# endernewton/tf-faster-rcnn

Measured on AMD Instinct MI355X. Metric: images/sec (600×1000) ResNet-101 Faster R-CNN at 1/2/4/8 MI355X, higher is better.
Workload: dtype f32 (operands, accumulators, results; GEMMs with Cin, Cout % 128 == 0 form each f32 product from two-piece fp16 operands with an exact power-of-two scale per 128-k block on the fp16 matrix pipe -- 3 MFMAs / product, dropped terms <= 3 * 2^-22, measured error vs float64 below the f32-MFMA kernel's; o

## Files before the change

include/frcnn_hip.h:

```cpp
#ifndef FRCNN_HIP_H_
#define FRCNN_HIP_H_
#include <stddef.h>
#include <stdint.h>

#ifdef __cplusplus
extern "C" {
#endif

#define FRCNN_OK 0
#define FRCNN_E_ARG (-1)
#define FRCNN_E_WS (-2)
#define FRCNN_E_UNSUPPORTED (-3)
#define FRCNN_E_HIP(e) (-(1000 + (int)(e)))

#define FRCNN_NMS_RULE_CPU 0
#define FRCNN_NMS_RULE_GPU 1

#define FRCNN_ACT_NONE 0
#define FRCNN_ACT_RELU 1
#define FRCNN_ACT_RELU6 2

#define FRCNN_ABI_VERSION 6
int frcnn_abi_version(void);
const char* frcnn_build_info(void);
// ... 128 lines not shown

int frcnn_gemm_batched_nt(const float* x_d, const float* w_d, float* y_d, int G, int M, int N, int K, void* stream);
size_t frcnn_gemm_x3_pack_bytes(int G, int N, int K);
int frcnn_gemm_x3_pack(const float* w_d, int G, int N, int K, void* planes_d, void* stream);
int frcnn_gemm_x3(const float* x_d, const void* planes_d, const float* bias_d, const float* res_d, float* y_d, int G, int M, int N,
                  int K, int act, int cfg, int terms, void* stream);
size_t frcnn_h2_planes_bytes(long long rows, int K);
int frcnn_h2_pack_w(const float* w_d, int G, int N, int K, void* planes_d, float* w_inv_d, void* stream);
int frcnn_h2_split(const float* x_d, long long M, int K, void* planes_d, float* inv_d, void* stream);
int frcnn_gemm_h2(const void* x_planes_d, const float* x_inv_d, const void* w_planes_d, const float* w_inv_d, const float* bias_d,
                  const float* res_d, const void* res_planes_d, const float* res_inv_d, float* y_d, void* y_planes_d, float* y_inv_d,
                  int G, int M, int N, int K, int act, int cfg, void* stream);
size_t frcnn_gemm_h2_mean_workspace_bytes(int G, int M, int N);
int frcnn_gemm_h2_mean(const void* x_planes_d, const float* x_inv_d, const void* w_planes_d, const float* w_inv_d, const float* bias_d,
                       const float* res_d, const void* res_planes_d, const float* res_inv_d, int G, int M, int N, int K, int act, int rows,
                       float* mean_out_d, void* ws, size_t ws_bytes, int cfg, void* stream);
int frcnn_winograd_filter_transform(const float* w_hwio, int Cin, int Cout, const float* scale, int m, float* u_out);
int frcnn_winograd_filter_transform_device(const float* w_packed_d, int Cout, int Cin, int m, int transpose_flip, float* u_d,
                                           void* stream);
int frcnn_winograd_input_transform(const float* x_d, int N, int H, int W, int C, int m, float* v_d, void* stream);
int frcnn_winograd_output_transform(const float* m_d, int N, int H, int W, int C, int m, const float* bias_d, int act, float* y_d,
                                    void* stream);
int frcnn_winograd7_filter_transform(const float* w_hwio, int Cin, int Cout, const float* scale, float* u_out);
int frcnn_winograd7_filter_transform_device(const float* w_packed_d, int Cout, int Cin, int transpose_flip, float* u_d, void* stream);
int frcnn_winograd7_input_transform(const float* x_d, int R, int C, float* v_d, void* stream);
int frcnn_winograd7_output_transform(const float* m_d, int R, int C, const float* bias_d, int act, float* y_d, void* stream);
int frcnn_winograd_input_transform_h2(const float* x_d, int N, int H, int W, int C, int m, void* v_planes_d, float* v_inv_d, void* stream);
int frcnn_winograd_output_transform_h2(const float* m_d, int N, int H, int W, int C, int m, const float* bias_d, int act, float* y_d,
                                       void* y_planes_d, float* y_inv_d, void* stream);
int frcnn_winograd7_input_transform_h2(const float* x_d, int R, int C, void* v_planes_d, float* v_inv_d, void* stream);
int frcnn_winograd7_output_transform_h2(const float* m_d, int R, int C, const float* bias_d, int act, float* y_d, void* y_planes_d,
                                        float* y_inv_d, void* stream);
int frcnn_pack_filter_hwio(const float* w_hwio, int KH, int KW, int Cin, int Cout, const float* scale, float* out);
int frcnn_maxpool_nhwc(const float* x_d, int N, int H, int W, int C, int k, int stride, int pad_top,
                       int pad_left, float* y_d, int OH, int OW, void* stream);
int frcnn_dwconv3x3_nhwc(const float* x_d, int N, int H, int W, int C, const float* w_d, const float* bias_d,
                         float* y_d, int OH, int OW, int stride, int pad_top, int pad_left, int act, void* stream);
int frcnn_dwconv3x3_nhwc_h2(const float* x_d, int N, int H, int W, int C, const float* w_d, const float* bias_d, float* y_d,
                            void* y_planes_d, float* y_inv_d, int OH, int OW, int stride, int pad_top, int pad_left, int act, void* stream);
int frcnn_spatial_mean(const float* x_d, int N, int HW, int C, float* y_d, void* stream);
int frcnn_softmax_rows(const float* x_d, int R, int C, int ld, float* y_d, void* stream);
int frcnn_rpn_softmax(const float* score_d, int HW, int A, int ld, float* prob_d, void* stream);
int frcnn_copy_cols(const float* src_d, int R, int ld_src, int col0, int cols, float* dst_d, int ld_dst, void* stream);

size_t frcnn_anchor_target_workspace_bytes(int H, int W, int A, int max_gt);
int frcnn_anchor_target_layer(const float* gt_boxes_d, int G, float im_h, float im_w, int H, int W, int A,
                              int feat_stride, const double* base_d, int rpn_batchsize, double fg_fraction,
                              double pos_overlap, double neg_overlap, long long seed, const double* opts, float* labels_d,
                              float* bbox_targets_d, float* inside_w_d, float* outside_w_d, void* ws,
                              size_t ws_bytes, void* stream);
int frcnn_anchor_target_layer_inject(const float* gt_boxes_d, int G, float im_h, float im_w, int H, int W, int A, int feat_stride,
                                     const double* base_d, int rpn_batchsize, double fg_fraction, double pos_overlap,
                                     double neg_overlap, const int* disable_d, int n_disable, const double* opts, float* labels_d,
                                     float* bbox_targets_d, float* inside_w_d, float* outside_w_d, void* ws, size_t ws_bytes,
                                     void* stream);
int frcnn_proposal_target_layer(const float* rpn_rois_d, const float* rpn_scores_d, int N, const float* gt_boxes_d,
                                int G, int num_classes, int batch_size, double fg_fraction, double fg_thresh,
                                double bg_thresh_hi, double bg_thresh_lo, const double* means4, const double* stds4,
                                long long seed, const double* opts, float* rois_d, float* roi_scores_d, float* labels_d,
                                float* bbox_targets_d, float* inside_w_d, float* outside_w_d, int* counts_d,
                                void* stream);
int frcnn_proposal_target_layer_dn(const float* rpn_rois_d, const float* rpn_scores_d, int max_rois, const int* num_rois_d,
                                   const float* gt_boxes_d, int G, int num_classes, int batch_size, double fg_fraction,
                                   double fg_thresh, double bg_thresh_hi, double bg_thresh_lo, const double* means4,
                                   const double* stds4, long long seed, const double* opts, float* rois_d, float* roi_scores_d,
                                   float* labels_d, float* bbox_targets_d, float* inside_w_d, float* outside_w_d, int* counts_d,
// ... 90 lines not shown
```

tf-faster-rcnn_amd/frcnn_hip/__init__.py:

```python
import ctypes
import os
from ctypes import c_double, c_float, c_int, c_longlong, c_size_t, c_ulonglong, c_void_p

_PKG = os.path.dirname(os.path.abspath(__file__))
LIB_PATH = os.path.join(_PKG, "libfrcnn_hip.so")
_lib = None

ABI_VERSION = 6
ACT_NONE, ACT_RELU, ACT_RELU6 = 0, 1, 2
NMS_RULE_CPU, NMS_RULE_GPU = 0, 1

_P = c_void_p
SIGNATURES = {
    "frcnn_abi_version": (c_int, []),
    "frcnn_build_info": (ctypes.c_char_p, []),
    "_nms": (None, [_P, _P, _P, c_int, c_int, c_float, c_int]),
    "frcnn_nms_workspace_bytes": (c_size_t, [c_int]),
    "frcnn_nms": (c_int, [_P, c_int, c_double, c_int, _P, _P, _P, c_size_t, _P]),
    "frcnn_nms_sorted": (c_int, [_P, c_int, c_int, c_double, c_int, _P, _P, _P, c_size_t, _P]),
    "frcnn_nms_rule": (c_int, [_P, c_int, c_double, c_int, c_int, _P, _P, _P, c_size_t, _P]),
    "frcnn_nms_sorted_rule": (c_int, [_P, c_int, c_int, c_double, c_int, c_int, _P, _P, _P, c_size_t, _P]),
    "frcnn_generate_anchors": (c_int, [c_int, _P, c_int, _P, c_int, _P]),
    "frcnn_generate_anchors_pre": (c_int, [c_int, c_int, c_int, _P, c_int, _P, _P]),
    "frcnn_proposal_workspace_bytes": (c_size_t, [c_int, c_int, c_int, c_int]),
# ... 41 lines not shown
    "frcnn_snappy_uncompress": (c_longlong, [_P, c_size_t, _P, c_size_t]),
    "frcnn_prep_image_shape": (c_int, [c_int, c_int, c_int, c_int, _P, _P, _P]),
    "frcnn_prep_image": (c_int, [_P, c_int, c_int, c_int, _P, c_double, _P, c_int, c_int, c_int, _P]),
    "frcnn_prep_image_batched": (c_int, [_P, c_int, c_int, c_int, c_int, _P, c_double, _P, c_int, c_int, c_int, _P]),
    "frcnn_prep_train_image": (c_int, [_P, c_int, c_int, c_int, c_int, _P, c_double, _P, c_int, c_int, c_int, _P, _P, c_int, _P, _P]),
    "frcnn_jpeg_info": (c_int, [_P, c_size_t, _P]),
    "frcnn_jpeg_coef_bytes": (c_size_t, [c_int, c_int, c_int, c_int, c_int]),
    "frcnn_jpeg_entropy_decode": (c_int, [_P, c_size_t, _P, c_size_t]),
    "frcnn_jpeg_pixels_host": (c_int, [_P, c_int, c_int, c_int, c_int, c_int, _P]),
    "frcnn_jpeg_workspace_bytes": (c_size_t, [c_int, c_int, c_int, c_int, c_int]),
    "frcnn_jpeg_pixels": (c_int, [_P, c_int, c_int, c_int, c_int, c_int, _P, _P, c_size_t, _P]),
    "frcnn_jpeg_quant_tables": (c_int, [c_int, _P]),
    "frcnn_jpeg_coefs": (c_int, [_P, c_int, c_int, c_int, c_int, c_int, _P, _P, c_size_t, _P]),
    "frcnn_jpeg_coefs_host": (c_int, [_P, c_int, c_int, c_int, c_int, c_int, _P]),
    "frcnn_jpeg_stream_bound": (c_size_t, [c_int, c_int, c_int, c_int]),
    "frcnn_jpeg_entropy_encode": (c_longlong, [_P, c_int, c_int, c_int, c_int, _P, c_size_t]),
    "frcnn_draw_detections": (c_int, [_P, c_int, c_int, _P, _P, c_int, c_float, c_int, c_int, _P, c_int, _P, c_int, c_int, _P, _P]),
    "frcnn_draw_detections_host": (c_int, [_P, c_int, c_int, _P, c_int, c_int, c_float, c_int, c_int, _P, c_int, _P, c_int, c_int, _P]),
    "frcnn_gemm_batched_nt": (c_int,[_P, _P, _P, c_int, c_int, c_int, c_int, _P]),
    "frcnn_winograd_filter_transform": (c_int, [_P, c_int, c_int, _P, c_int, _P]),
    "frcnn_winograd_filter_transform_device": (c_int, [_P, c_int, c_int, c_int, c_int, _P, _P]),
    "frcnn_winograd_input_transform": (c_int, [_P, c_int, c_int, c_int, c_int, c_int, _P, _P]),
    "frcnn_winograd_output_transform": (c_int, [_P, c_int, c_int, c_int, c_int, c_int, _P, c_int, _P, _P]),
    "frcnn_winograd7_filter_transform": (c_int, [_P, c_int, c_int, _P, _P]),
    "frcnn_winograd7_filter_transform_device": (c_int, [_P, c_int, c_int, c_int, _P, _P]),
    "frcnn_winograd7_input_transform": (c_int, [_P, c_int, c_int, _P, _P]),
    "frcnn_winograd7_output_transform": (c_int, [_P, c_int, c_int, _P, c_int, _P, _P]),
    "frcnn_winograd_input_transform_h2": (c_int, [_P, c_int, c_int, c_int, c_int, c_int, _P, _P, _P]),
    "frcnn_winograd_output_transform_h2": (c_int, [_P, c_int, c_int, c_int, c_int, c_int, _P, c_int, _P, _P, _P, _P]),
    "frcnn_winograd7_input_transform_h2": (c_int, [_P, c_int, c_int, _P, _P, _P]),
    "frcnn_winograd7_output_transform_h2": (c_int, [_P, c_int, c_int, _P, c_int, _P, _P, _P, _P]),
    "frcnn_set_tuning": (c_int, [c_int, c_int]),
    "frcnn_pack_filter_hwio": (c_int, [_P, c_int, c_int, c_int, c_int, _P, _P]),
    "frcnn_maxpool_nhwc": (c_int, [_P, c_int, c_int, c_int, c_int, c_int, c_int, c_int, c_int, _P, c_int, c_int, _P]),
    "frcnn_dwconv3x3_nhwc": (c_int, [_P, c_int, c_int, c_int, c_int, _P, _P, _P, c_int, c_int, c_int, c_int, c_int, c_int, _P]),
    "frcnn_dwconv3x3_nhwc_h2": (c_int, [_P, c_int, c_int, c_int, c_int, _P, _P, _P, _P, _P, c_int, c_int, c_int, c_int, c_int, c_int, _P]),
    "frcnn_spatial_mean": (c_int, [_P, c_int, c_int, c_int, _P, _P]),
    "frcnn_softmax_rows": (c_int, [_P, c_int, c_int, c_int, _P, _P]),
    "frcnn_rpn_softmax": (c_int, [_P, c_int, c_int, c_int, _P, _P]),
    "frcnn_copy_cols": (c_int, [_P, c_int, c_int, c_int, c_int, _P, c_int, _P]),
    "frcnn_anchor_target_workspace_bytes": (c_size_t, [c_int, c_int, c_int, c_int]),
    "frcnn_anchor_target_layer": (c_int, [_P, c_int, c_float, c_float, c_int, c_int, c_int, c_int, _P, c_int, c_double, c_double,
                                          c_double, c_longlong, _P, _P, _P, _P, _P, _P, c_size_t, _P]),
    "frcnn_anchor_target_layer_inject": (c_int, [_P, c_int, c_float, c_float, c_int, c_int, c_int, c_int, _P, c_int, c_double, c_double,
                                                 c_double, _P, c_int, _P, _P, _P, _P, _P, _P, c_size_t, _P]),
    "frcnn_proposal_target_layer_inject": (c_int, [_P, _P, c_int, _P, c_int, c_int, c_int, _P, c_int, _P, _P, _P, _P, _P, _P, _P, _P, _P, _P]),
    "frcnn_proposal_target_layer": (c_int, [_P, _P, c_int, _P, c_int, c_int, c_int, c_double, c_double, c_double, c_double, _P, _P,
                                            c_longlong, _P, _P, _P, _P, _P, _P, _P, _P, _P]),
    "frcnn_proposal_target_layer_dn": (c_int, [_P, _P, c_int, _P, _P, c_int, c_int, c_int, c_double, c_double, c_double, c_double, _P, _P,
                                               c_longlong, _P, _P, _P, _P, _P, _P, _P, _P, _P]),
    "frcnn_loss_workspace_bytes": (c_size_t, [c_longlong]),
    "frcnn_softmax_ce_loss": (c_int, [_P, _P, c_int, c_int, c_int, c_int, c_int, _P, _P, _P, c_size_t, _P]),
    "frcnn_smooth_l1_loss": (c_int, [_P, _P, _P, _P, c_longlong, c_float, c_float, _P, _P, _P, c_size_t, _P]),
    "frcnn_transpose_pad": (c_int, [_P, c_int, c_int, _P, c_int, _P]),
    "frcnn_im2col_t": (c_int, [_P, c_int, c_int, c_int, c_int, c_int, c_int, c_int, c_int, c_int, c_int, c_int, _P, c_int, _P]),
    "frcnn_flip_transpose_filter": (c_int, [_P, c_int, c_int, c_int, c_int, _P, _P]),
    "frcnn_conv2d_dgrad_strided": (c_int, [_P, c_int, c_int, c_int, c_int, _P, c_int, c_int, c_int, c_int, c_int, c_int, _P, c_int,
                                           c_int, c_int, _P]),
    "frcnn_conv2d_wgrad_supported": (c_int, [c_int, c_int]),
    "frcnn_conv2d_wgrad_workspace_bytes": (c_size_t, [c_int, c_int, c_int, c_int, c_int, c_int, c_int]),
    "frcnn_conv2d_wgrad": (c_int, [_P, _P, c_int, c_int, c_int, c_int, c_int, c_int, c_int, c_int, c_int, c_int, c_int, c_int, _P, _P,
                                   c_size_t, _P]),
    "frcnn_conv2d_wgrad_set_plan": (None, [c_int, c_int]),
    "frcnn_conv2d_wgrad_h2_workspace_bytes": (c_size_t, [c_int, c_int, c_int, c_int, c_int, c_int, c_int]),
    "frcnn_conv2d_wgrad_h2": (c_int, [_P, _P, c_int, c_int, c_int, c_int, c_int, c_int, c_int, c_int, c_int, c_int, c_int, c_int, _P, _P,
                                      c_size_t, _P]),
# ... 78 lines not shown
```

tf-faster-rcnn_amd/frcnn_hip/build.py:

```python
import glob
import os
import subprocess
import sys
from concurrent.futures import ThreadPoolExecutor

PKG = os.path.dirname(os.path.abspath(__file__))
ROOT = os.path.dirname(os.path.dirname(PKG))
CSRC = os.path.join(os.path.dirname(PKG), "csrc")
OBJ = os.path.join(CSRC, "build")
LIB = os.path.join(PKG, "libfrcnn_hip.so")
SOURCES = ["detect_kernels.hip", "conv_igemm.hip", "dense_misc.hip", "train_kernels.hip", "backward_kernels.hip", "winograd.hip", "winograd7.hip", "preproc.hip", "gemm_x3.hip", "gemm_h2.hip", "wgrad_tn.hip", "wgrad_h2.hip", "coco_eval.hip", "jpeg_decode.hip", "summary_stats.hip", "jpeg_encode.hip", "draw.hip"]
FLAGS = ["-O3", "-std=c++17", "--offload-arch=gfx950", "-fPIC", "-ffp-contract=off",
         "-I" + os.path.join(ROOT, "include"), "-I" + CSRC]


def _hipcc():
    for c in (os.environ.get("HIPCC"), "/opt/rocm/bin/hipcc", "hipcc"):
        if c and (os.path.isabs(c) and os.path.exists(c) or not os.path.isabs(c)):
            return c
    return "hipcc"


def _stale(target, deps):
    if not os.path.exists(target):
        return True
    t = os.path.getmtime(target)
    return any(os.path.getmtime(d) > t for d in deps)


def build(force=False, verbose=False):
    os.makedirs(OBJ, exist_ok=True)
    hdrs = [os.path.join(ROOT, "include", "frcnn_hip.h")] + sorted(glob.glob(os.path.join(CSRC, "*.h")))
    objs, jobs = [], []
    for s in SOURCES:
        src, obj = os.path.join(CSRC, s), os.path.join(OBJ, s.replace(".hip", ".o"))
        objs.append(obj)
        if force or _stale(obj, [src] + hdrs):
            jobs.append([_hipcc()] + FLAGS + ["-c", src, "-o", obj])

    def run(cmd):
        if verbose:
            print(" ".join(cmd))
        subprocess.check_call(cmd)
    with ThreadPoolExecutor(max_workers=4) as ex:
# ... 9 lines not shown
```

tf-faster-rcnn_amd/frcnn_hip/ops.py:

```python
import ctypes

import numpy as np
import torch

import frcnn_hip as _binding
from . import ACT_NONE, NMS_RULE_CPU, call, check, lib

_ws_cache = {}
ws_scope = "default"

_scope_stack = [(None, None, None)]


def active_store(owner, default=None):
    o, _, store = _scope_stack[-1]
    return store if store is not None and (owner is None or o is owner) else default


def scope_depth():
    return len(_scope_stack) - 1


class unscoped(object):

    def __enter__(self):
        _scope_stack.append(_scope_stack[0])

    def __exit__(self, *exc):
        _scope_stack.pop()


stream_pin = None


def _stream():
    return stream_pin if stream_pin is not None else ctypes.c_void_p(torch.cuda.current_stream().cuda_stream)


class pinned_stream(object):
# ... 367 lines not shown
def conv2d(x, w_packed, bias, KH, KW, stride=1, pad=(0, 0, 0, 0), act=ACT_NONE, residual=None, res_stride=1,
           fold_w=False, out=None, mask=None):
    _chk(x), _chk(w_packed)
    N, H, W, Cin = x.shape
    Cout = w_packed.shape[0]
    OH = conv_out_size(H, KH, stride, pad[0], pad[1])
    OW = conv_out_size(W, KW, stride, pad[2], pad[3])
    out = _empty((N, OH, OW, Cout), dtype=torch.float32, device=x.device) if out is None else out
    RH = RW = 0
    if residual is not None:
        _chk(residual)
        RH, RW = residual.shape[1], residual.shape[2]
    nb = lib().frcnn_conv2d_workspace_bytes(N, OH, OW, Cout, KH, KW, Cin, 1 if fold_w else 0) if split_k else 0
    if mask is not None:
        _chk(mask)
        assert not fold_w and mask.numel() == out.numel()
        ws = workspace(nb, x.device, "conv_splitk") if nb else None
        call("frcnn_conv2d_nhwc_masked_ws", _ptr(x), N, H, W, Cin, _ptr(w_packed), _ptr(bias), _ptr(residual), RH, RW,
             int(res_stride), _ptr(out), OH, OW, Cout, KH, KW, int(stride), int(pad[0]), int(pad[2]), int(act), _ptr(mask),
             _ptr(ws), ws.numel() if nb else 0, _stream())
        return out
    if nb:
        ws = workspace(nb, x.device, "conv_splitk")
        call("frcnn_conv2d_nhwc_ws", _ptr(x), N, H, W, Cin, _ptr(w_packed), _ptr(bias), _ptr(residual), RH, RW,
             int(res_stride), _ptr(out), OH, OW, Cout, KH, KW, int(stride), int(pad[0]), int(pad[2]), int(act),
             1 if fold_w else 0, _ptr(ws), ws.numel(), _stream())
        return out
    call("frcnn_conv2d_nhwc", _ptr(x), N, H, W, Cin, _ptr(w_packed), _ptr(bias), _ptr(residual), RH, RW,
         int(res_stride), _ptr(out), OH, OW, Cout, KH, KW, int(stride), int(pad[0]), int(pad[2]), int(act),
         1 if fold_w else 0, _stream())
    return out


def prep_image_shape(h, w, target_size, max_size):
    sc, oh, ow = ctypes.c_double(), ctypes.c_int(), ctypes.c_int()
    call("frcnn_prep_image_shape", int(h), int(w), int(target_size), int(max_size), ctypes.byref(sc), ctypes.byref(oh),
         ctypes.byref(ow))
    return sc.value, oh.value, ow.value


def prep_image(im_d, pixel_means, im_scale, out_hw, out=None, out_c=4):
    assert im_d.is_cuda and im_d.is_contiguous() and im_d.dim() == 3 and im_d.shape[2] == 3
    assert im_d.dtype in (torch.uint8, torch.float32)
    h, w = im_d.shape[:2]
    OH, OW = out_hw
    out = _empty((1, OH, OW, out_c), dtype=torch.float32, device=im_d.device) if out is None else out
    assert out.shape == (1, OH, OW, out_c)
    means = (ctypes.c_double * 3)(*[float(v) for v in np.asarray(pixel_means, dtype=np.float64).reshape(-1)[:3]])
    call("frcnn_prep_image", _ptr(im_d), 1 if im_d.dtype == torch.float32 else 0, h, w, means, float(im_scale), _ptr(out), OH, OW,
         int(out_c), _stream())
    return out


def prep_image_batched(ims_d, pixel_means, im_scale, out_hw, out=None, out_c=4):
    assert ims_d.is_cuda and ims_d.is_contiguous() and ims_d.dim() == 4 and ims_d.shape[3] == 3 and ims_d.shape[0] >= 1
    assert ims_d.dtype in (torch.uint8, torch.float32)
    B, h, w = ims_d.shape[:3]
    OH, OW = out_hw
    out = _empty((B, OH, OW, out_c), dtype=torch.float32, device=ims_d.device) if out is None else out
    assert out.shape == (B, OH, OW, out_c) and out.is_contiguous() and out.dtype == torch.float32
    means = (ctypes.c_double * 3)(*[float(v) for v in np.asarray(pixel_means, dtype=np.float64).reshape(-1)[:3]])
    call("frcnn_prep_image_batched", _ptr(ims_d), 1 if ims_d.dtype == torch.float32 else 0, B, h, w, means, float(im_scale), _ptr(out), OH,
         OW, int(out_c), _stream())
    return out


# ... 823 lines not shown
```

tf-faster-rcnn_amd/lib/model/config.py:

```python
import ast
import os
import os.path as osp

import numpy as np


class AttrDict(dict):

    def __init__(self, d=None, **kw):
        super().__init__()
        for k, v in dict(d or {}, **kw).items():
            self[k] = v

    def __setitem__(self, k, v):
        if isinstance(v, dict) and not isinstance(v, AttrDict):
            v = AttrDict(v)
        super().__setitem__(k, v)

    def __getattr__(self, k):
        try:
            return self[k]
        except KeyError:
            raise AttributeError(k)

    __setattr__ = __setitem__


_TRAIN = dict(
    LEARNING_RATE=0.001, MOMENTUM=0.9, WEIGHT_DECAY=0.0001, GAMMA=0.1, STEPSIZE=[30000], DISPLAY=10,
    DOUBLE_BIAS=True, TRUNCATED=False, BIAS_DECAY=False, USE_GT=False, ASPECT_GROUPING=False,
    SNAPSHOT_KEPT=3, SUMMARY_INTERVAL=180, SCALES=(600,), MAX_SIZE=1000, IMS_PER_BATCH=1, BATCH_SIZE=128,
    FG_FRACTION=0.25, FG_THRESH=0.5, BG_THRESH_HI=0.5, BG_THRESH_LO=0.1, USE_FLIPPED=True, BBOX_REG=True,
    BBOX_THRESH=0.5, SNAPSHOT_ITERS=5000, SNAPSHOT_PREFIX='res101_faster_rcnn', BBOX_NORMALIZE_TARGETS=True,
    BBOX_INSIDE_WEIGHTS=(1.0, 1.0, 1.0, 1.0), BBOX_NORMALIZE_TARGETS_PRECOMPUTED=True,
    BBOX_NORMALIZE_MEANS=(0.0, 0.0, 0.0, 0.0), BBOX_NORMALIZE_STDS=(0.1, 0.1, 0.2, 0.2), PROPOSAL_METHOD='gt',
    HAS_RPN=True, RPN_POSITIVE_OVERLAP=0.7, RPN_NEGATIVE_OVERLAP=0.3, RPN_CLOBBER_POSITIVES=False,
    RPN_FG_FRACTION=0.5, RPN_BATCHSIZE=256, RPN_NMS_THRESH=0.7, RPN_PRE_NMS_TOP_N=12000,
    RPN_POST_NMS_TOP_N=2000, RPN_BBOX_INSIDE_WEIGHTS=(1.0, 1.0, 1.0, 1.0), RPN_POSITIVE_WEIGHT=-1.0,
    USE_ALL_GT=True)

_TEST = dict(
    SCALES=(600,), MAX_SIZE=1000, NMS=0.3, SVM=False, BBOX_REG=True, HAS_RPN=False, PROPOSAL_METHOD='gt',
    RPN_NMS_THRESH=0.7, RPN_PRE_NMS_TOP_N=6000, RPN_POST_NMS_TOP_N=300, MODE='nms', RPN_TOP_N=5000)

__C = AttrDict(
    TRAIN=_TRAIN, TEST=_TEST,
    RESNET=dict(MAX_POOL=False, FIXED_BLOCKS=1),
    MOBILENET=dict(REGU_DEPTH=False, FIXED_LAYERS=5, WEIGHT_DECAY=0.00004, DEPTH_MULTIPLIER=1.),
    PIXEL_MEANS=np.array([[[102.9801, 115.9465, 122.7717]]]), RNG_SEED=3,
    ROOT_DIR=osp.abspath(osp.join(osp.dirname(__file__), '..', '..')),
    MATLAB='matlab', EXP_DIR='default', USE_GPU_NMS=True, USE_E2E_TF=False, POOLING_MODE='crop', POOLING_SIZE=7,
    ANCHOR_SCALES=[8, 16, 32], ANCHOR_RATIOS=[0.5, 1, 2], RPN_CHANNELS=512,
    HIP=dict(WINOGRAD=True, WINOGRAD_MIN_CIN=64, WINOGRAD_M=4, WINOGRAD_F2_SCOPES=("block1", "block2"), WINOGRAD_DIRECT_SCOPES=(),
             WINOGRAD_TRAIN=True, WINOGRAD_DGRAD=True,
             WINOGRAD_7X7=True, FUSE_TAIL_MEAN=True, MFMA_X3=True,
             MFMA_H2=True, H2_LAZY_SPLIT=True, H2_MIN_TILES=150, H2_TRAIN_MIN_TILES=320, H2_TRUNK_PLANES=True, H2_TILE_CFG=-1,
             X3_TILE_CFG=-1, H2_TRAIN=True, WGRAD_STREAM=2, WGRAD_TN=True, WGRAD_H2=True, PREP_STREAM=True, TRAIN_REPLAY=True, TRAIN_PICK_STREAMS=6,
             GRAPH_CACHE_SHAPES=4, TRAIN_CACHE_SHAPES=16, JPEG_DEVICE=False, TEST_BATCH_IMAGES=1))
__C.DATA_DIR = osp.abspath(osp.join(__C.ROOT_DIR, 'data'))
cfg = __C


def get_output_dir(imdb, weights_filename):
    outdir = osp.abspath(osp.join(__C.ROOT_DIR, 'output', __C.EXP_DIR, imdb.name))
    outdir = osp.join(outdir, 'default' if weights_filename is None else weights_filename)
    os.makedirs(outdir, exist_ok=True)
    return outdir


def get_output_tb_dir(imdb, weights_filename):
    outdir = osp.abspath(osp.join(__C.ROOT_DIR, 'tensorboard', __C.EXP_DIR, imdb.name))
    outdir = osp.join(outdir, 'default' if weights_filename is None else weights_filename)
    os.makedirs(outdir, exist_ok=True)
    return outdir


_NULLABLE_KEYS = ("H2_TRAIN_MIN_TILES",)


def _merge_a_into_b(a, b):
    if not isinstance(a, dict):
        return
    for k, v in a.items():
        if k not in b:
            raise KeyError('{} is not a valid config key'.format(k))
        old = b[k]
        if type(old) is not type(v) and not (isinstance(old, dict) and isinstance(v, dict)):
            if isinstance(old, np.ndarray):
                v = np.array(v, dtype=old.dtype)
            elif isinstance(old, tuple) and isinstance(v, list):
                v = tuple(v)
# ... 45 lines not shown
```

tf-faster-rcnn_amd/lib/nets/network.py:

```python
import collections

import numpy as np
import torch

from frcnn_hip import ACT_NONE, ACT_RELU, NMS_RULE_CPU, NMS_RULE_GPU, ops
from frcnn_hip.runtime import VarSpec
from model.config import cfg


class Network(object):
    def __init__(self):
        self._predictions = {}
        self._losses = {}
        self._anchor_targets = {}
        self._proposal_targets = {}
        self._layers = {}
        self._act_summaries = []
        self._variables_to_fix = {}
        self._feat_stride = [16, ]
        self._scope = "network"
        self._sess = None
        self._image = None
        self._im_info = None
        self._var_specs = collections.OrderedDict()
# ... 520 lines not shown
        A = self._num_anchors
        self._var_specs.clear()
        self._declare_backbone()
        hc = self._head_channels()
        self._declare_conv_bias(self._scope + "/rpn_conv/3x3", 3, 3, hc, cfg.RPN_CHANNELS, 0.01)
        self._declare_conv_bias(self._scope + "/rpn_cls_score", 1, 1, cfg.RPN_CHANNELS, 2 * A, 0.01)
        self._declare_conv_bias(self._scope + "/rpn_bbox_pred", 1, 1, cfg.RPN_CHANNELS, 4 * A, 0.01)
        tc = self._tail_channels()
        self._var(self._scope + "/cls_score/weights", (tc, num_classes), "normal", 0.01)
        self._var(self._scope + "/cls_score/biases", (num_classes,), "zeros")
        self._var(self._scope + "/bbox_pred/weights", (tc, 4 * num_classes), "normal", 0.001)
        self._var(self._scope + "/bbox_pred/biases", (4 * num_classes,), "zeros")
        names = ["rois", "rpn_cls_score", "rpn_cls_prob", "rpn_bbox_pred", "cls_score", "cls_prob", "bbox_pred"]
        return {k: k for k in names}

    def _stage_image(self, sess, image, im_info=None):
        if isinstance(image, np.ndarray):
            image = torch.from_numpy(np.ascontiguousarray(image, dtype=np.float32))
        B, H, W, C = image.shape
        if im_info is None:
            buf = sess.buf(self._tag + "/image", (B, H, W, 4), zero=True)
        else:
            with self.shape_scope(sess, (B, H, W, 4), im_info):
                buf = sess.buf(self._tag + "/image", (B, H, W, 4), zero=True)
        buf[..., :C].copy_(image, non_blocking=True)
        return buf

    def graph_key(self, image_shape, im_info):
        c = cfg[self._mode]
        return (self._tag, self._scope, self._num_classes, self._anchor_scales, self._anchor_ratios, bool(cfg.RESNET.MAX_POOL),
                bool(cfg.USE_GPU_NMS), tuple(int(v) for v in image_shape), (float(im_info[0]), float(im_info[1])), self._mode, cfg.TEST.MODE, self._fuse_tail_entry,
                c.RPN_PRE_NMS_TOP_N, c.RPN_POST_NMS_TOP_N, c.RPN_NMS_THRESH, cfg.TEST.RPN_TOP_N, cfg.POOLING_SIZE,
                bool(cfg.HIP.WINOGRAD), int(cfg.HIP.WINOGRAD_MIN_CIN), int(cfg.HIP.WINOGRAD_M), tuple(cfg.HIP.WINOGRAD_F2_SCOPES),
                tuple(cfg.HIP.WINOGRAD_DIRECT_SCOPES), bool(cfg.HIP.WINOGRAD_7X7), bool(cfg.HIP.FUSE_TAIL_MEAN), bool(cfg.HIP.MFMA_X3), bool(cfg.USE_E2E_TF),
                bool(cfg.HIP.MFMA_H2), bool(cfg.HIP.H2_LAZY_SPLIT), int(cfg.HIP.H2_MIN_TILES), bool(cfg.HIP.H2_TRUNK_PLANES), int(cfg.HIP.H2_TILE_CFG), int(cfg.HIP.X3_TILE_CFG), bool(cfg.HIP.H2_TRAIN))

    def shape_scope(self, sess, image_shape, im_info):
        return sess.shape_scope(self.graph_key(image_shape, im_info), group=("graphs", self._tag), cap=int(cfg.HIP.GRAPH_CACHE_SHAPES))

    def forward_device(self, sess, image_d, im_info, use_graph=True):
        self._sess = sess
        self._image = image_d
        self._im_info = (float(im_info[0]), float(im_info[1]), float(im_info[2]))
        sess.prepared.wait_planes()
        ops.ws_scope = self._tag
        key = self.graph_key(image_d.shape, self._im_info)
        cur = torch.cuda.current_stream(sess.device)
        with self.shape_scope(sess, image_d.shape, self._im_info):
            if not use_graph or sess.profile is not None:
                sess.flops_last_forward = 0
                self._build_network(self._mode == "TRAIN")
                return self._predictions
            if key not in sess.graphs:
                with torch.cuda.stream(sess.stream):
                    sess.stream.wait_stream(cur)
                    sess.flops_last_forward = 0
                    self._build_network(False)
                    sess.stream.synchronize()
                    flops = sess.flops_last_forward
                    g = ops.Graph().capture(lambda: self._build_network(False))
                    sess.stream.synchronize()
                sess.graphs[key] = (g, dict(self._predictions), self._num_rois, flops, self._rois_per_image, image_d)
            g, preds, num, flops, per, captured = sess.graphs[key]
            self._predictions, self._num_rois, sess.flops_last_forward, self._rois_per_image = dict(preds), num, flops, per
            if captured.data_ptr() != image_d.data_ptr():
                captured.copy_(image_d, non_blocking=True)
            g.launch()
# ... 316 lines not shown
```

tf-faster-rcnn_amd/lib/nets/resnet_v1.py:

```python
from frcnn_hip import ACT_NONE, ACT_RELU, ops
from model.config import cfg
from nets.network import Network

BN_EPS = 1e-5


def _same_pad(k, stride):
    total = k - 1
    beg = total // 2
    return (beg, total - beg, beg, total - beg)


class resnetv1(Network):
    _rgb_first_conv = "/conv1"
    _trainable_on_device = True
    def __init__(self, num_layers=50):
        Network.__init__(self)
        self._feat_stride = [16, ]
        self._feat_compress = [1. / float(self._feat_stride[0]), ]
        self._num_layers = num_layers
        self._scope = 'resnet_v1_%d' % num_layers
        self._decide_blocks()

    def _decide_blocks(self):
# ... 41 lines not shown
            r = self._conv(r, prefix + "/conv2", 3, stride, pad, act=ACT_RELU, bn_eps=BN_EPS, emit_h2=True, want_f32=False)
            if self._h2_input(r) is not None:
                return self._conv1x1_mean(r, prefix + "/conv3", mean_rows, act=ACT_RELU, bn_eps=BN_EPS, residual=shortcut)
            x = self._conv(r, prefix + "/conv3", 1, 1, act=ACT_RELU, bn_eps=BN_EPS, residual=shortcut, res_stride=1)
            out = self._sess.buf(self._tag + "/fc7", (x.shape[0], x.shape[-1]))
            return self._sess.mark("op:spatial_mean", 0, lambda: ops.spatial_mean(x, out=out), nbytes=4 * (x.numel() + out.numel()))
        c3_h2 = res_stride == 1 and self._h2_eligible(M3, depth, base, 1, prefix + "/conv3")
        r = self._conv(r, prefix + "/conv2", 3, stride, pad, act=ACT_RELU, bn_eps=BN_EPS, emit_h2=c3_h2, want_f32=not c3_h2)
        return self._conv(r, prefix + "/conv3", 1, 1, act=ACT_RELU, bn_eps=BN_EPS, residual=shortcut, res_stride=res_stride,
                          emit_h2=emit_out, want_f32=f32_out)

    def _trunk_planes_only(self, rows, base, next_stride, next_prefix=None):
        depth = 4 * base
        return (bool(cfg.HIP.H2_TRUNK_PLANES) and next_stride == 1
                and self._h2_eligible(rows, base, depth, 1, None if next_prefix is None else next_prefix + "/conv1")
                and self._h2_eligible(rows, depth, base, 1, None if next_prefix is None else next_prefix + "/conv3"))

    def _run_blocks(self, x, blocks, emit_last=True):
        for bi, (name, base, n_units, stride) in enumerate(blocks):
            for u in range(1, n_units + 1):
                s_u = stride if u == n_units else 1
                N, H, W, _ = x.shape
                rows = N * ops.conv_out_size(H, 3, s_u, 1, 1) * ops.conv_out_size(W, 3, s_u, 1, 1) if s_u > 1 else N * H * W
                planes_only = u < n_units and self._trunk_planes_only(rows, base, stride if u + 1 == n_units else 1,
                                                                       "%s/%s/unit_%d/bottleneck_v1" % (self._scope, name, u + 1))
                x = self._bottleneck(x, "%s/%s/unit_%d/bottleneck_v1" % (self._scope, name, u), base, s_u,
                                     emit_out=emit_last or u < n_units or bi + 1 < len(blocks), f32_out=not planes_only)
        return x

    def _crop_pool_layer(self, bottom, rois, name):
        return self._crop_pool(bottom, rois, name, max_pool=bool(cfg.RESNET.MAX_POOL))

    def _build_base(self):
        net = self._conv(self._image, self._scope + "/conv1", 7, 2, _same_pad(7, 2), act=ACT_RELU, bn_eps=BN_EPS,
                         fold_w=True, real_cin=3)
        N, H, W, C = net.shape
        out = self._sess.buf(self._tag + "/pool1", (N, ops.conv_out_size(H, 3, 2, 1, 1), ops.conv_out_size(W, 3, 2, 1, 1), C))
        self._sess.mark("op:maxpool", 0, lambda: ops.maxpool(net, 3, 2, (1, 1, 1, 1), out=out), nbytes=4 * (net.numel() + out.numel()))
        return self._wrote(out)

    def _image_to_head(self, is_training, reuse=None):
        assert (0 <= cfg.RESNET.FIXED_BLOCKS <= 3)
        net_conv = self._run_blocks(self._build_base(), self._blocks[0:3])
        self._act_summaries.append(net_conv)
        self._layers['head'] = net_conv
        return net_conv

    def _fused_tail_maps(self, net_conv):
        name = self._blocks[-1][0]
        prefix = "%s/%s/unit_1/bottleneck_v1" % (self._scope, name)
        sc_map = self._conv(net_conv, prefix + "/shortcut", 1, 1, act=ACT_NONE, bn_eps=BN_EPS, no_bias=True)
        c1_map = self._conv(net_conv, prefix + "/conv1", 1, 1, act=ACT_NONE, bn_eps=BN_EPS, no_bias=True)
        return sc_map, c1_map

    def _fused_tail_entry(self, net_conv, rois):
        sess, P = self._sess, cfg.POOLING_SIZE
        name, base, n_units, stride = self._blocks[-1]
        prefix = "%s/%s/unit_1/bottleneck_v1" % (self._scope, name)
        R = rois.shape[0]
        sc_map, c1_map = self._fused_tail_maps(net_conv)
        b_sc = sess.conv_info[prefix + "/shortcut"]["b"]
        b_c1 = sess.conv_info[prefix + "/conv1"]["b"]
        fs = float(self._feat_stride[0])
        sc_out = sess.buf(self._tag + "/" + prefix + "/shortcut_crop", (R, P, P, sc_map.shape[-1]))
        c1_out = sess.buf(self._tag + "/" + prefix + "/conv1_crop", (R, P, P, c1_map.shape[-1]))
        shortcut = self._crop_images(sc_map, rois, sc_out, bias=b_sc, act=ACT_NONE)
        r = self._crop_images(c1_map, rois, c1_out, bias=b_c1, act=ACT_RELU)
        c3_h2 = self._h2_eligible(R * P * P, 4 * base, base, 1, prefix + "/conv3")
        r = self._conv(r, prefix + "/conv2", 3, 1, (1, 1, 1, 1), act=ACT_RELU, bn_eps=BN_EPS, emit_h2=c3_h2, want_f32=not c3_h2)
        x = self._conv(r, prefix + "/conv3", 1, 1, act=ACT_RELU, bn_eps=BN_EPS, residual=shortcut, res_stride=1, emit_h2=n_units >= 2,
                       want_f32=not (n_units >= 2 and self._trunk_planes_only(R * P * P, base, stride if n_units == 2 else 1,
# ... 35 lines not shown
```

Baseline: 549.3.

## Fuse ResNet stem 7x7 stride-2 conv with 3x3 max-pool in one kernel

Adds a dedicated HIP kernel that computes the 7x7/s2 conv1 (Cin padded to 4, Cout 64, ReLU) with f32 MFMA on an LDS-resident, parity-split input patch. The 3x3/s2 max-pool is applied from LDS staging, so only the pooled output is written. This removes the full-resolution conv1 activation round-trip to global memory and one kernel launch in TEST mode. The cost is recomputing the overlapping conv halo per tile and a fixed-shape kernel that only supports this exact configuration.

```diff
diff --git a/include/frcnn_hip.h b/include/frcnn_hip.h
--- a/include/frcnn_hip.h
+++ b/include/frcnn_hip.h
@@ -184,6 +184,8 @@
 int frcnn_winograd7_output_transform_h2(const float* m_d, int R, int C, const float* bias_d, int act, float* y_d, void* y_planes_d,
                                         float* y_inv_d, void* stream);
 int frcnn_pack_filter_hwio(const float* w_hwio, int KH, int KW, int Cin, int Cout, const float* scale, float* out);
+int frcnn_stem7x7s2_pool3x3s2(const float* x_d, int N, int H, int W, int Cin, const float* w_d, const float* bias_d, int Cout,
+                              int KH, int KW, int stride, int act, float* y_d, int POH, int POW, void* stream);
 int frcnn_maxpool_nhwc(const float* x_d, int N, int H, int W, int C, int k, int stride, int pad_top,
                        int pad_left, float* y_d, int OH, int OW, void* stream);
 int frcnn_dwconv3x3_nhwc(const float* x_d, int N, int H, int W, int C, const float* w_d, const float* bias_d,
diff --git a/tf-faster-rcnn_amd/csrc/stem.hip b/tf-faster-rcnn_amd/csrc/stem.hip
--- /dev/null
+++ b/tf-faster-rcnn_amd/csrc/stem.hip
@@ -0,0 +1,174 @@
+#include "common.h"
+
+namespace {
+
+constexpr int TP_H = 7, TP_W = 8;
+constexpr int CR = 2 * TP_H + 1, CC = 2 * TP_W + 1;
+constexpr int CPIX = CR * CC;
+constexpr int PR = 2 * CR + 5, PC = 2 * CC + 5;
+constexpr int YH = (PR + 1) / 2, XH = (PC + 1) / 2;
+constexpr int RS = 49;
+constexpr int PYP = YH * RS;
+constexpr int CP = 2 * PYP;
+constexpr int PATCH = 3 * CP;
+constexpr int KSTEPS = 74;
+constexpr int FS = 65;
+constexpr int FILT = 2 * KSTEPS * FS;
+constexpr int STAGE = CPIX * 64;
+constexpr int LDS_FLOATS = (PATCH + FILT > STAGE) ? PATCH + FILT : STAGE;
+constexpr int THREADS = 256;
+
+static_assert(CPIX <= 256 && CPIX > 224, "8 row blocks of 32");
+static_assert(RS % 32 == CC % 32 && RS >= 2 * XH, "conflict-free rows");
+static_assert(LDS_FLOATS * 4 * 2 <= 160 * 1024, "two workgroups per CU");
+
+__host__ __device__ constexpr int tap_off(int c, int kh, int kw) {
+  return c * CP + (kh & 1) * PYP + (kh >> 1) * RS + (kw & 1) * XH + (kw >> 1);
+}
+struct Tap {
+  int kh, kw, c;
+};
+__host__ __device__ constexpr Tap chain_tap(int i) {
+  const int kh = i / 21, r = i % 21;
+  return i == 147 ? Tap{6, 7, 2} : (r < 18 ? Tap{kh, 2 * (r / 6) + (r & 1), (r % 6) / 2} : Tap{kh, 6, r - 18});
+}
+__host__ __device__ constexpr int chain_off(int i) { return tap_off(chain_tap(i).c, chain_tap(i).kh, chain_tap(i).kw); }
+__device__ __forceinline__ int filt_row(int kh, int kw, int c) { return kh * 21 + (kw < 6 ? (kw >> 1) * 6 + 2 * c + (kw & 1) : 18 + c); }
+constexpr int NDIST = 5;
+constexpr int DIST[NDIST] = {XH, CP, CP - XH, 1 - XH - 2 * CP, PYP - 3 - 2 * CP};
+__host__ __device__ constexpr int step_off(int j) { return chain_off(2 * j); }
+__host__ __device__ constexpr int step_group(int j) {
+  const int d = chain_off(2 * j + 1) - chain_off(2 * j);
+  return d == XH ? 0 : d == CP ? 1 : d == CP - XH ? 2 : d == 1 - XH - 2 * CP ? 3 : d == PYP - 3 - 2 * CP ? 4 : -1;
+}
+__host__ __device__ constexpr bool steps_ok() {
+  for (int j = 0; j < KSTEPS; ++j)
+    if (step_group(j) < 0) return false;
+  return true;
+}
+static_assert(steps_ok(), "every pair of consecutive taps lies one of the DIST constants apart");
+
+typedef float f32x16 __attribute__((ext_vector_type(16)));
+
+__global__ __launch_bounds__(THREADS, 2) void k_stem7_pool(const float4* __restrict__ x, int H, int W, const float4* __restrict__ w,
+                                                           const float* __restrict__ bias, float* __restrict__ y, int OH, int OW,
+                                                           int POH, int POW) {
+  __shared__ __attribute__((aligned(16))) float lds[LDS_FLOATS];
+  float* const patch = lds;
+  float* const filt = lds + PATCH;
+  const int tid = threadIdx.x, lane = tid & 63, wave = tid >> 6;
+  const int img = blockIdx.z;
+  const int p0 = blockIdx.y * TP_H, q0 = blockIdx.x * TP_W;
+  const int cy0 = 2 * p0 - 1, cx0 = 2 * q0 - 1;
+  const int iy0 = 2 * cy0 - 3, ix0 = 2 * cx0 - 3;
+
+  const float4* xi = x + (size_t)img * H * W;
+  constexpr int PITEMS = 2 * YH * 2 * XH, PTRIPS = (PITEMS + THREADS - 1) / THREADS, FTRIPS = 64 * 7 * 8 / THREADS;
+  static_assert(FTRIPS * THREADS == 64 * 7 * 8, "filter trips");
+  float4 pv[PTRIPS], fv[FTRIPS];
+#pragma unroll
+  for (int u = 0; u < PTRIPS; ++u) {
+    const int i = tid + u * THREADS, py = i / (2 * XH), px = i - py * (2 * XH);
+    const int iy = iy0 + py, ix = ix0 + px;
+    pv[u] = make_float4(0.f, 0.f, 0.f, 0.f);
+    if (py < PR && px < PC && (unsigned)iy < (unsigned)H && (unsigned)ix < (unsigned)W) pv[u] = xi[(size_t)iy * W + ix];
+  }
+#pragma unroll
+  for (int u = 0; u < FTRIPS; ++u) fv[u] = w[tid + u * THREADS];
+#pragma unroll
+  for (int u = 0; u < PTRIPS; ++u) {
+    const int i = tid + u * THREADS, py = i / (2 * XH), px = i - py * (2 * XH);
+    if (i < PITEMS) {
+      float* d = patch + (py & 1) * PYP + (py >> 1) * RS + (px & 1) * XH + (px >> 1);
+      d[0] = pv[u].x, d[CP] = pv[u].y, d[2 * CP] = pv[u].z;
+    }
+  }
+#pragma unroll
+  for (int u = 0; u < FTRIPS; ++u) {
+    const int i = tid + u * THREADS, n = i / 56, r = i - n * 56, kh = r >> 3, kw = r & 7;
+    if (kw < 7) {
+      filt[filt_row(kh, kw, 0) * FS + n] = fv[u].x;
+      filt[filt_row(kh, kw, 1) * FS + n] = fv[u].y;
+      filt[filt_row(kh, kw, 2) * FS + n] = fv[u].z;
+    }
+  }
+  if (tid < 64) filt[(2 * KSTEPS - 1) * FS + tid] = 0.f;
+  __syncthreads();
+
+  const int half = lane >> 5, col = lane & 31;
+  f32x16 acc[2][2];
+#pragma unroll
+  for (int i = 0; i < 2; ++i)
+#pragma unroll
+    for (int j = 0; j < 2; ++j)
+#pragma unroll
+      for (int r = 0; r < 16; ++r) acc[i][j][r] = 0.f;
+  {
+    int m0 = (2 * wave) * 32 + col, m1 = m0 + 32;
+    m1 = m1 < CPIX ? m1 : CPIX - 1;
+    const int pix0 = (m0 / CC) * RS + (m0 % CC), pix1 = (m1 / CC) * RS + (m1 % CC);
+    const float* pb = filt + half * FS + col;
+    const float *a0g[NDIST], *a1g[NDIST];
+#pragma unroll
+    for (int g = 0; g < NDIST; ++g) a0g[g] = patch + pix0 + half * DIST[g], a1g[g] = patch + pix1 + half * DIST[g];
+#pragma unroll
+    for (int j = 0; j < KSTEPS; ++j) {
+      const int g = step_group(j), off = step_off(j);
+      const float a0 = a0g[g][off], a1 = a1g[g][off];
+      const float b0 = pb[j * 2 * FS], b1 = pb[j * 2 * FS + 32];
+      acc[0][0] = __builtin_amdgcn_mfma_f32_32x32x2f32(a0, b0, acc[0][0], 0, 0, 0);
+      acc[0][1] = __builtin_amdgcn_mfma_f32_32x32x2f32(a0, b1, acc[0][1], 0, 0, 0);
+      acc[1][0] = __builtin_amdgcn_mfma_f32_32x32x2f32(a1, b0, acc[1][0], 0, 0, 0);
+      acc[1][1] = __builtin_amdgcn_mfma_f32_32x32x2f32(a1, b1, acc[1][1], 0, 0, 0);
+    }
+  }
+  __syncthreads();
+
+  float* const stage = lds;
+  const float bz0 = bias ? bias[col] : 0.f, bz1 = bias ? bias[32 + col] : 0.f;
+#pragma unroll
+  for (int i = 0; i < 2; ++i)
+#pragma unroll
+    for (int r = 0; r < 16; ++r) {
+      const int m = (2 * wave + i) * 32 + (r & 3) + 8 * (r >> 2) + 4 * half;
+      if (m < CPIX) {
+        const int oy = m / CC, ox = m - oy * CC;
+        const bool in = (unsigned)(cy0 + oy) < (unsigned)OH && (unsigned)(cx0 + ox) < (unsigned)OW;
+        stage[m * 64 + col] = in ? act_relu(acc[i][0][r] + bz0) : 0.f;
+        stage[m * 64 + 32 + col] = in ? act_relu(acc[i][1][r] + bz1) : 0.f;
+      }
+    }
+  __syncthreads();
+
+  const float4* st4 = (const float4*)stage;
+  for (int i = tid; i < TP_H * TP_W * 16; i += THREADS) {
+    const int n4 = i & 15, pp = i >> 4, pl = pp / TP_W, ql = pp - pl * TP_W;
+    const int p = p0 + pl, q = q0 + ql;
+    if (p >= POH || q >= POW) continue;
+    float4 m = make_float4(-INFINITY, -INFINITY, -INFINITY, -INFINITY);
+#pragma unroll
+    for (int dy = 0; dy < 3; ++dy)
+#pragma unroll
+      for (int dx = 0; dx < 3; ++dx) {
+        const float4 v = st4[((2 * pl + dy) * CC + 2 * ql + dx) * 16 + n4];
+        m = make_float4(fmaxf(m.x, v.x), fmaxf(m.y, v.y), fmaxf(m.z, v.z), fmaxf(m.w, v.w));
+      }
+    ((float4*)y)[(((size_t)img * POH + p) * POW + q) * 16 + n4] = m;
+  }
+}
+
+}
+
+extern "C" int frcnn_stem7x7s2_pool3x3s2(const float* x_d, int N, int H, int W, int Cin, const float* w_d, const float* bias_d, int Cout,
+                                         int KH, int KW, int stride, int act, float* y_d, int POH, int POW, void* stream) {
+  if (!x_d || !w_d || !y_d || N <= 0 || H <= 0 || W <= 0 || Cin <= 0 || Cout <= 0 || KH <= 0 || KW <= 0 || stride <= 0) return FRCNN_E_ARG;
+  if (Cin != 4 || Cout != 64 || KH != 7 || KW != 7 || stride != 2 || act != FRCNN_ACT_RELU) return FRCNN_E_UNSUPPORTED;
+  const int OH = (H - 1) / 2 + 1, OW = (W - 1) / 2 + 1;
+  if (POH != (OH - 1) / 2 + 1 || POW != (OW - 1) / 2 + 1) return FRCNN_E_ARG;
+  const int tx = cdiv(POW, TP_W), ty = cdiv(POH, TP_H);
+  if (N > 65535 || ty > 65535) return FRCNN_E_UNSUPPORTED;
+  hipLaunchKernelGGL(k_stem7_pool, dim3(tx, ty, N), dim3(THREADS), 0, (hipStream_t)stream, (const float4*)x_d, H, W,
+                     (const float4*)w_d, bias_d, y_d, OH, OW, POH, POW);
+  LAUNCH_CHECK();
+  return FRCNN_OK;
+}
diff --git a/tf-faster-rcnn_amd/frcnn_hip/__init__.py b/tf-faster-rcnn_amd/frcnn_hip/__init__.py
--- a/tf-faster-rcnn_amd/frcnn_hip/__init__.py
+++ b/tf-faster-rcnn_amd/frcnn_hip/__init__.py
@@ -97,6 +97,7 @@
     "frcnn_winograd7_output_transform_h2": (c_int, [_P, c_int, c_int, _P, c_int, _P, _P, _P, _P]),
     "frcnn_set_tuning": (c_int, [c_int, c_int]),
     "frcnn_pack_filter_hwio": (c_int, [_P, c_int, c_int, c_int, c_int, _P, _P]),
+    "frcnn_stem7x7s2_pool3x3s2": (c_int, [_P, c_int, c_int, c_int, c_int, _P, _P, c_int, c_int, c_int, c_int, c_int, _P, c_int, c_int, _P]),
     "frcnn_maxpool_nhwc": (c_int, [_P, c_int, c_int, c_int, c_int, c_int, c_int, c_int, c_int, _P, c_int, c_int, _P]),
     "frcnn_dwconv3x3_nhwc": (c_int, [_P, c_int, c_int, c_int, c_int, _P, _P, _P, c_int, c_int, c_int, c_int, c_int, c_int, _P]),
     "frcnn_dwconv3x3_nhwc_h2": (c_int, [_P, c_int, c_int, c_int, c_int, _P, _P, _P, _P, _P, c_int, c_int, c_int, c_int, c_int, c_int, _P]),
diff --git a/tf-faster-rcnn_amd/frcnn_hip/build.py b/tf-faster-rcnn_amd/frcnn_hip/build.py
--- a/tf-faster-rcnn_amd/frcnn_hip/build.py
+++ b/tf-faster-rcnn_amd/frcnn_hip/build.py
@@ -9,7 +9,7 @@
 CSRC = os.path.join(os.path.dirname(PKG), "csrc")
 OBJ = os.path.join(CSRC, "build")
 LIB = os.path.join(PKG, "libfrcnn_hip.so")
-SOURCES = ["detect_kernels.hip", "conv_igemm.hip", "dense_misc.hip", "train_kernels.hip", "backward_kernels.hip", "winograd.hip", "winograd7.hip", "preproc.hip", "gemm_x3.hip", "gemm_h2.hip", "wgrad_tn.hip", "wgrad_h2.hip", "coco_eval.hip", "jpeg_decode.hip", "summary_stats.hip", "jpeg_encode.hip", "draw.hip"]
+SOURCES = ["detect_kernels.hip", "conv_igemm.hip", "stem.hip", "dense_misc.hip", "train_kernels.hip", "backward_kernels.hip", "winograd.hip", "winograd7.hip", "preproc.hip", "gemm_x3.hip", "gemm_h2.hip", "wgrad_tn.hip", "wgrad_h2.hip", "coco_eval.hip", "jpeg_decode.hip", "summary_stats.hip", "jpeg_encode.hip", "draw.hip"]
 FLAGS = ["-O3", "-std=c++17", "--offload-arch=gfx950", "-fPIC", "-ffp-contract=off",
          "-I" + os.path.join(ROOT, "include"), "-I" + CSRC]
 
diff --git a/tf-faster-rcnn_amd/frcnn_hip/ops.py b/tf-faster-rcnn_amd/frcnn_hip/ops.py
--- a/tf-faster-rcnn_amd/frcnn_hip/ops.py
+++ b/tf-faster-rcnn_amd/frcnn_hip/ops.py
@@ -4,7 +4,7 @@
 import torch
 
 import frcnn_hip as _binding
-from . import ACT_NONE, NMS_RULE_CPU, call, check, lib
+from . import ACT_NONE, ACT_RELU, NMS_RULE_CPU, call, check, lib
 
 _ws_cache = {}
 ws_scope = "default"
@@ -438,6 +438,18 @@
     return out
 
 
+def stem_conv_pool(x, w_packed, bias, out=None, KH=7, KW=7, stride=2, act=ACT_RELU):
+    _chk(x), _chk(w_packed)
+    N, H, W, Cin = x.shape
+    Cout = w_packed.shape[0]
+    OH, OW = conv_out_size(H, 7, 2, 3, 3), conv_out_size(W, 7, 2, 3, 3)
+    POH, POW = conv_out_size(OH, 3, 2, 1, 1), conv_out_size(OW, 3, 2, 1, 1)
+    out = _empty((N, POH, POW, Cout), dtype=torch.float32, device=x.device) if out is None else out
+    call("frcnn_stem7x7s2_pool3x3s2", _ptr(x), N, H, W, Cin, _ptr(w_packed), _ptr(bias), Cout, int(KH), int(KW), int(stride), int(act),
+         _ptr(out), POH, POW, _stream())
+    return out
+
+
 def prep_image_shape(h, w, target_size, max_size):
     sc, oh, ow = ctypes.c_double(), ctypes.c_int(), ctypes.c_int()
     call("frcnn_prep_image_shape", int(h), int(w), int(target_size), int(max_size), ctypes.byref(sc), ctypes.byref(oh),
diff --git a/tf-faster-rcnn_amd/lib/model/config.py b/tf-faster-rcnn_amd/lib/model/config.py
--- a/tf-faster-rcnn_amd/lib/model/config.py
+++ b/tf-faster-rcnn_amd/lib/model/config.py
@@ -56,7 +56,7 @@
              WINOGRAD_7X7=True, FUSE_TAIL_MEAN=True, MFMA_X3=True,
              MFMA_H2=True, H2_LAZY_SPLIT=True, H2_MIN_TILES=150, H2_TRAIN_MIN_TILES=320, H2_TRUNK_PLANES=True, H2_TILE_CFG=-1,
              X3_TILE_CFG=-1, H2_TRAIN=True, WGRAD_STREAM=2, WGRAD_TN=True, WGRAD_H2=True, PREP_STREAM=True, TRAIN_REPLAY=True, TRAIN_PICK_STREAMS=6,
-             GRAPH_CACHE_SHAPES=4, TRAIN_CACHE_SHAPES=16, JPEG_DEVICE=False, TEST_BATCH_IMAGES=1))
+             GRAPH_CACHE_SHAPES=4, TRAIN_CACHE_SHAPES=16, JPEG_DEVICE=False, TEST_BATCH_IMAGES=1, STEM_POOL_FUSED=True))
 __C.DATA_DIR = osp.abspath(osp.join(__C.ROOT_DIR, 'data'))
 cfg = __C
 
diff --git a/tf-faster-rcnn_amd/lib/nets/network.py b/tf-faster-rcnn_amd/lib/nets/network.py
--- a/tf-faster-rcnn_amd/lib/nets/network.py
+++ b/tf-faster-rcnn_amd/lib/nets/network.py
@@ -576,7 +576,7 @@
                 bool(cfg.USE_GPU_NMS), tuple(int(v) for v in image_shape), (float(im_info[0]), float(im_info[1])), self._mode, cfg.TEST.MODE, self._fuse_tail_entry,
                 c.RPN_PRE_NMS_TOP_N, c.RPN_POST_NMS_TOP_N, c.RPN_NMS_THRESH, cfg.TEST.RPN_TOP_N, cfg.POOLING_SIZE,
                 bool(cfg.HIP.WINOGRAD), int(cfg.HIP.WINOGRAD_MIN_CIN), int(cfg.HIP.WINOGRAD_M), tuple(cfg.HIP.WINOGRAD_F2_SCOPES),
-                tuple(cfg.HIP.WINOGRAD_DIRECT_SCOPES), bool(cfg.HIP.WINOGRAD_7X7), bool(cfg.HIP.FUSE_TAIL_MEAN), bool(cfg.HIP.MFMA_X3), bool(cfg.USE_E2E_TF),
+                tuple(cfg.HIP.WINOGRAD_DIRECT_SCOPES), bool(cfg.HIP.WINOGRAD_7X7), bool(cfg.HIP.STEM_POOL_FUSED), bool(cfg.HIP.FUSE_TAIL_MEAN), bool(cfg.HIP.MFMA_X3), bool(cfg.USE_E2E_TF),
                 bool(cfg.HIP.MFMA_H2), bool(cfg.HIP.H2_LAZY_SPLIT), int(cfg.HIP.H2_MIN_TILES), bool(cfg.HIP.H2_TRUNK_PLANES), int(cfg.HIP.H2_TILE_CFG), int(cfg.HIP.X3_TILE_CFG), bool(cfg.HIP.H2_TRAIN))
 
     def shape_scope(self, sess, image_shape, im_info):
diff --git a/tf-faster-rcnn_amd/lib/nets/resnet_v1.py b/tf-faster-rcnn_amd/lib/nets/resnet_v1.py
--- a/tf-faster-rcnn_amd/lib/nets/resnet_v1.py
+++ b/tf-faster-rcnn_amd/lib/nets/resnet_v1.py
@@ -97,11 +97,23 @@
         return self._crop_pool(bottom, rois, name, max_pool=bool(cfg.RESNET.MAX_POOL))
 
     def _build_base(self):
+        if self._mode == "TEST" and cfg.HIP.STEM_POOL_FUSED:
+            sess, scope, x = self._sess, self._scope + "/conv1", self._image
+            w, b = sess.conv_params(scope, bn_eps=BN_EPS, fold_w=True)
+            N, H, W, _ = x.shape
+            OH, OW = ops.conv_out_size(H, 7, 2, 3, 3), ops.conv_out_size(W, 7, 2, 3, 3)
+            out = sess.buf(self._tag + "/pool1", (N, ops.conv_out_size(OH, 3, 2, 1, 1), ops.conv_out_size(OW, 3, 2, 1, 1), w.shape[0]))
+            self._need_f32(x)
+            sess.mark("conv:" + scope, 2 * N * OH * OW * w.shape[0] * 7 * 7 * 3, lambda: ops.stem_conv_pool(x, w, b, out=out),
+                      nbytes=4 * (x.numel() + w.numel() + out.numel()))
+            self._layers["pool1"] = out
+            return self._wrote(out)
         net = self._conv(self._image, self._scope + "/conv1", 7, 2, _same_pad(7, 2), act=ACT_RELU, bn_eps=BN_EPS,
                          fold_w=True, real_cin=3)
         N, H, W, C = net.shape
         out = self._sess.buf(self._tag + "/pool1", (N, ops.conv_out_size(H, 3, 2, 1, 1), ops.conv_out_size(W, 3, 2, 1, 1), C))
         self._sess.mark("op:maxpool", 0, lambda: ops.maxpool(net, 3, 2, (1, 1, 1, 1), out=out), nbytes=4 * (net.numel() + out.numel()))
+        self._layers["pool1"] = out
         return self._wrote(out)
 
     def _image_to_head(self, is_training, reuse=None):
```

Result: no change. 554.5, median of 6 (+1.0%).
